# AlibabaResearch/efficientteacher

Measured on AMD Instinct MI355X. Metric: SSOD images/sec (teacher+student step) YOLOv5l 640px, higher is better.
Workload: dtype bf16

## Files before the change

### efficientteacher_amd/csrc/spatial.hip

```cpp
#include "et_host.h"

template <typename T>
__global__ __launch_bounds__(256) void pack_input_kernel(const float* __restrict__ x, T* __restrict__ y, int C, int HW, long long total) {
    const unsigned iu = blockIdx.x * 256u + threadIdx.x;
    if (iu >= total) return;
    const long long i = iu, b = iu / (unsigned)HW, hw = iu - (unsigned)b * (unsigned)HW;
    T v[8];
#pragma unroll
    for (int c = 0; c < 8; ++c) v[c] = et_elem<T>::st(c < C ? x[(b * C + c) * HW + hw] : 0.f);
    T* d = y + i * 8;
#pragma unroll
    for (int c = 0; c < 8; ++c) d[c] = v[c];
}

template <typename T>
__global__ __launch_bounds__(256) void pack_input_u8_kernel(const uint8_t* __restrict__ x, T* __restrict__ y, int C, int HW,
                                                            long long total, float scale) {
    const unsigned iu = blockIdx.x * 256u + threadIdx.x;
    if (iu >= total) return;
    const long long i = iu, b = iu / (unsigned)HW, hw = iu - (unsigned)b * (unsigned)HW;
    T v[8];
#pragma unroll
    for (int c = 0; c < 8; ++c) v[c] = et_elem<T>::st(c < C ? (float)x[(b * C + c) * HW + hw] / scale : 0.f);
    T* d = y + i * 8;
#pragma unroll
    for (int c = 0; c < 8; ++c) d[c] = v[c];
}

template <typename IN, typename T = uint16_t>
__global__ __launch_bounds__(256) void pack_input4_bf16_kernel(const IN* __restrict__ x, T* __restrict__ y, int C, int HW4,
                                                               long long total4, float scale) {
    const unsigned qu = blockIdx.x * 256u + threadIdx.x;
    if (qu >= total4) return;
    const unsigned b = qu / (unsigned)HW4, h4 = qu - b * (unsigned)HW4;
    float v[4][4];
#pragma unroll
    for (int c = 0; c < 4; ++c) {
#pragma unroll
        for (int j = 0; j < 4; ++j) v[c][j] = 0.f;
        if (c < C) {
            const long long off = ((long long)b * C + c) * HW4 * 4 + (long long)h4 * 4;
            if constexpr (sizeof(IN) == 4) {
                const float4 t = *(const float4*)((const float*)x + off);
                v[c][0] = t.x; v[c][1] = t.y; v[c][2] = t.z; v[c][3] = t.w;
            } else {
                const unsigned w = *(const unsigned*)((const uint8_t*)x + off);
#pragma unroll
                for (int j = 0; j < 4; ++j) v[c][j] = (float)((w >> (8 * j)) & 0xffu) / scale;
            }
        }
    }
    T* const d = y + ((long long)b * HW4 * 4 + (long long)h4 * 4) * 8;
#pragma unroll
    for (int j = 0; j < 4; ++j)
        *(uint4*)(d + j * 8) = make_uint4(et_lp<T>::pack(v[0][j], v[1][j]), et_lp<T>::pack(v[2][j], v[3][j]), 0u, 0u);
}

template <typename T> struct PV;
template <> struct PV<float> {
    static constexpr int N = 4;
    __device__ static __forceinline__ void load(const float* p, float (&v)[4]) { const float4 t = *(const float4*)p; v[0] = t.x; v[1] = t.y; v[2] = t.z; v[3] = t.w; }
    __device__ static __forceinline__ void store(float* p, const float (&v)[4]) { *(float4*)p = make_float4(v[0], v[1], v[2], v[3]); }
};
template <typename T> struct PVlp {
    static constexpr int N = 8;
    __device__ static __forceinline__ void load(const T* p, float (&v)[8]) {
        const uint4 t = *(const uint4*)p;
        const unsigned w[4] = {t.x, t.y, t.z, t.w};
#pragma unroll
        for (int i = 0; i < 4; ++i) { v[2 * i] = et_lp<T>::lo(w[i]); v[2 * i + 1] = et_lp<T>::hi(w[i]); }
    }
    __device__ static __forceinline__ void store(T* p, const float (&v)[8]) {
        *(uint4*)p = make_uint4(et_lp<T>::pack(v[0], v[1]), et_lp<T>::pack(v[2], v[3]), et_lp<T>::pack(v[4], v[5]), et_lp<T>::pack(v[6], v[7]));
    }
};
template <> struct PV<uint16_t> : PVlp<uint16_t> {};
template <> struct PV<et_f16> : PVlp<et_f16> {};

template <typename T>
__global__ __launch_bounds__(256) void maxpool5_fwd_kernel(const T* __restrict__ x, int ldx, T* __restrict__ y, int ldy,
                                                           unsigned char* __restrict__ idx, int H, int W, int CV, long long total) {
    constexpr int N = PV<T>::N;
    const unsigned iu = blockIdx.x * 256u + threadIdx.x;
    if (iu >= total) return;
    const unsigned pu = iu / (unsigned)CV, tu = pu / (unsigned)W;
    const int cv = (int)(iu - pu * (unsigned)CV);
    const long long p = pu;
    const int ox = (int)(pu - tu * (unsigned)W);
    const long long b = tu / (unsigned)H;
    const int oy = (int)(tu - (unsigned)b * (unsigned)H);
    float best[N];
    unsigned char bi[N];
#pragma unroll
    for (int k = 0; k < N; ++k) { best[k] = -INFINITY; bi[k] = 0; }
    for (int ky = 0; ky < 5; ++ky) {
        const int iy = oy + ky - 2;
        if ((unsigned)iy >= (unsigned)H) continue;
        for (int kx = 0; kx < 5; ++kx) {
            const int ix = ox + kx - 2;
            if ((unsigned)ix >= (unsigned)W) continue;
            float v[N];
            PV<T>::load(x + ((b * H + iy) * W + ix) * ldx + cv * N, v);
#pragma unroll
            for (int k = 0; k < N; ++k)
                if (v[k] > best[k]) { best[k] = v[k]; bi[k] = (unsigned char)(ky * 5 + kx); }
        }
    }
    PV<T>::store(y + p * ldy + cv * N, best);
    unsigned char* ip = idx + (p * CV + cv) * N;
#pragma unroll
    for (int k = 0; k < N; ++k) ip[k] = bi[k];
}

template <typename T>
__global__ __launch_bounds__(256) void maxpool5_bwd_kernel(const T* __restrict__ dy, int lddy, const unsigned char* __restrict__ idx,
                                                           const T* __restrict__ base, int ldb, T* __restrict__ dx, int lddx,
                                                           int H, int W, int CV, long long total) {
    constexpr int N = PV<T>::N;
    const unsigned iu = blockIdx.x * 256u + threadIdx.x;
    if (iu >= total) return;
    const unsigned pu = iu / (unsigned)CV, tu = pu / (unsigned)W;
    const int cv = (int)(iu - pu * (unsigned)CV);
    const long long p = pu;
    const int ix = (int)(pu - tu * (unsigned)W);
    const long long b = tu / (unsigned)H;
    const int iy = (int)(tu - (unsigned)b * (unsigned)H);
    float acc[N];
    if (base) PV<T>::load(base + p * ldb + cv * N, acc);
    else {
#pragma unroll
        for (int k = 0; k < N; ++k) acc[k] = 0.f;
    }
    for (int ky = 0; ky < 5; ++ky) {
        const int oy = iy - ky + 2;
        if ((unsigned)oy >= (unsigned)H) continue;
        for (int kx = 0; kx < 5; ++kx) {
            const int ox = ix - kx + 2;
            if ((unsigned)ox >= (unsigned)W) continue;
            const long long q = (b * H + oy) * W + ox;
            float g[N];
            PV<T>::load(dy + q * lddy + cv * N, g);
            const unsigned char* ip = idx + (q * CV + cv) * N;
            const unsigned char code = (unsigned char)(ky * 5 + kx);
#pragma unroll
            for (int k = 0; k < N; ++k)
                if (ip[k] == code) acc[k] += g[k];
        }
    }
    PV<T>::store(dx + p * lddx + cv * N, acc);
}

template <typename T>
__global__ __launch_bounds__(256) void upsample2x_fwd_kernel(const T* __restrict__ x, int ldx, T* __restrict__ y, int ldy, int H, int W,
                                                             int CV, long long total) {
    const unsigned iu = blockIdx.x * 256u + threadIdx.x;
    if (iu >= total) return;
    const unsigned pu = iu / (unsigned)CV, tu = pu / (unsigned)(2 * W);
    const int cv = (int)(iu - pu * (unsigned)CV);
    const long long p = pu;
    const int ox = (int)(pu - tu * (unsigned)(2 * W));
    const long long b = tu / (unsigned)(2 * H);
    const int oy = (int)(tu - (unsigned)b * (unsigned)(2 * H));
    const uint4 v = *(const uint4*)((const char*)(x + ((b * H + (oy >> 1)) * W + (ox >> 1)) * ldx) + (size_t)cv * 16);
    *(uint4*)((char*)(y + p * ldy) + (size_t)cv * 16) = v;
}

template <typename T>
__global__ __launch_bounds__(256) void upsample2x_bwd_kernel(const T* __restrict__ dy, int lddy, T* __restrict__ dx, int lddx, int H, int W,
                                                             int CV, long long total, int accumulate) {
    constexpr int N = PV<T>::N;
    const unsigned iu = blockIdx.x * 256u + threadIdx.x;
    if (iu >= total) return;
    const unsigned pu = iu / (unsigned)CV, tu = pu / (unsigned)W;
    const int cv = (int)(iu - pu * (unsigned)CV);
    const long long p = pu;
    const int w = (int)(pu - tu * (unsigned)W);
    const long long b = tu / (unsigned)H;
    const int h = (int)(tu - (unsigned)b * (unsigned)H);
    float acc[N];
    if (accumulate) PV<T>::load(dx + p * lddx + cv * N, acc);
    else {
#pragma unroll
        for (int k = 0; k < N; ++k) acc[k] = 0.f;
    }
#pragma unroll
    for (int d = 0; d < 4; ++d) {
        const long long q = (b * 2 * H + (2 * h + (d >> 1))) * 2 * W + (2 * w + (d & 1));
        float g[N];
        PV<T>::load(dy + q * lddy + cv * N, g);
#pragma unroll
        for (int k = 0; k < N; ++k) acc[k] += g[k];
    }
    PV<T>::store(dx + p * lddx + cv * N, acc);
}

extern "C" int et_pack_input(const float* x_nchw, void* y_nhwc8, int dtype, int B, int C, int H, int W, et_stream_t stream) {
    if (!x_nchw || !y_nhwc8) return -1;
    if (B <= 0 || C <= 0 || C > 8 || H <= 0 || W <= 0) return -2;
    const long long total = (long long)B * H * W;
    if (total >= (1ll << 31)) return -2;
    return with_dtype(dtype, [&](auto t) {
        using T = typename decltype(t)::type;
        const bool quads = et_is_lp<T>::value && C <= 4 && (H * W) % 4 == 0 && ((((uintptr_t)x_nchw) | ((uintptr_t)y_nhwc8)) & 15) == 0;
        if constexpr (et_is_lp<T>::value) {
            if (quads)
                hipLaunchKernelGGL((pack_input4_bf16_kernel<float, T>), dim3(et_cdiv(total / 4, 256)), dim3(256), 0, (hipStream_t)stream, x_nchw,
                                   (T*)y_nhwc8, C, H * W / 4, total / 4, 1.0f);
        }
        if (!quads)
            hipLaunchKernelGGL((pack_input_kernel<T>), dim3(et_cdiv(total, 256)), dim3(256), 0, (hipStream_t)stream, x_nchw, (T*)y_nhwc8, C, H * W, total);
        ET_CHECK_LAUNCH();
        return 0;
    });
}

extern "C" int et_pack_input_u8(const uint8_t* x_nchw, void* y_nhwc8, int dtype, int B, int C, int H, int W, float norm_scale,
                                et_stream_t stream) {
    if (!x_nchw || !y_nhwc8) return -1;
    if (B <= 0 || C <= 0 || C > 8 || H <= 0 || W <= 0 || !(norm_scale > 0.f)) return -2;
    const long long total = (long long)B * H * W;
    if (total >= (1ll << 31)) return -2;
    return with_dtype(dtype, [&](auto t) {
        using T = typename decltype(t)::type;
        const bool quads = et_is_lp<T>::value && C <= 4 && (H * W) % 4 == 0 && (((uintptr_t)x_nchw) & 3) == 0 && (((uintptr_t)y_nhwc8) & 15) == 0;
        if constexpr (et_is_lp<T>::value) {
            if (quads)
                hipLaunchKernelGGL((pack_input4_bf16_kernel<uint8_t, T>), dim3(et_cdiv(total / 4, 256)), dim3(256), 0, (hipStream_t)stream, x_nchw,
                                   (T*)y_nhwc8, C, H * W / 4, total / 4, norm_scale);
        }
        if (!quads)
            hipLaunchKernelGGL((pack_input_u8_kernel<T>), dim3(et_cdiv(total, 256)), dim3(256), 0, (hipStream_t)stream, x_nchw, (T*)y_nhwc8, C, H * W, total,
                               norm_scale);
        ET_CHECK_LAUNCH();
        return 0;
    });
}

extern "C" int et_maxpool5_fwd(const void* x, int ldx, void* y, int ldy, uint8_t* argmax, int dtype, int B, int H, int W, int C,
                               et_stream_t stream) {
    if (!x || !y || !argmax) return -1;
    const int vec = et_vec(dtype), CV = C / vec;
    if (B <= 0 || !et_whole_vecs(vec, C, ldx, ldy)) return -2;
    const long long total = (long long)B * H * W * CV;
    if (total >= (1ll << 31)) return -2;
    return with_dtype(dtype, [&](auto t) {
        using T = typename decltype(t)::type;
        hipLaunchKernelGGL((maxpool5_fwd_kernel<T>), dim3(et_cdiv(total, 256)), dim3(256), 0, (hipStream_t)stream, (const T*)x, ldx, (T*)y, ldy, argmax,
                           H, W, CV, total);
        ET_CHECK_LAUNCH();
        return 0;
    });
}

extern "C" int et_maxpool5_bwd(const void* dy, int lddy, const uint8_t* argmax, const void* base, int ldb, void* dx, int lddx,
                               int dtype, int B, int H, int W, int C, et_stream_t stream) {
    if (!dy || !dx || !argmax) return -1;
    const int vec = et_vec(dtype), CV = C / vec;
    if (B <= 0 || !et_whole_vecs(vec, C, lddy, lddx) || (base && ldb % vec)) return -2;
    const long long total = (long long)B * H * W * CV;
    if (total >= (1ll << 31)) return -2;
    return with_dtype(dtype, [&](auto t) {
        using T = typename decltype(t)::type;
        hipLaunchKernelGGL((maxpool5_bwd_kernel<T>), dim3(et_cdiv(total, 256)), dim3(256), 0, (hipStream_t)stream, (const T*)dy, lddy, argmax,
                           (const T*)base, ldb, (T*)dx, lddx, H, W, CV, total);
        ET_CHECK_LAUNCH();
        return 0;
    });
}

extern "C" int et_upsample2x_fwd(const void* x, int ldx, void* y, int ldy, int dtype, int B, int H, int W, int C, et_stream_t stream) {
    if (!x || !y) return -1;
    const int vec = et_vec(dtype), CV = C / vec;
    if (B <= 0 || !et_whole_vecs(vec, C, ldx, ldy)) return -2;
    const long long total = (long long)B * 4 * H * W * CV;
    if (total >= (1ll << 31)) return -2;
    return with_dtype(dtype, [&](auto t) {
        using T = typename decltype(t)::type;
        hipLaunchKernelGGL((upsample2x_fwd_kernel<T>), dim3(et_cdiv(total, 256)), dim3(256), 0, (hipStream_t)stream, (const T*)x, ldx, (T*)y, ldy, H, W,
                           CV, total);
        ET_CHECK_LAUNCH();
        return 0;
    });
}

extern "C" int et_upsample2x_bwd(const void* dy, int lddy, void* dx, int lddx, int dtype, int B, int H, int W, int C, int accumulate,
                                 et_stream_t stream) {
    if (!dy || !dx) return -1;
    const int vec = et_vec(dtype), CV = C / vec;
    if (B <= 0 || !et_whole_vecs(vec, C, lddy, lddx)) return -2;
    const long long total = (long long)B * H * W * CV;
    if (total >= (1ll << 31)) return -2;
    return with_dtype(dtype, [&](auto t) {
        using T = typename decltype(t)::type;
        hipLaunchKernelGGL((upsample2x_bwd_kernel<T>), dim3(et_cdiv(total, 256)), dim3(256), 0, (hipStream_t)stream, (const T*)dy, lddy, (T*)dx, lddx,
                           H, W, CV, total, accumulate);
        ET_CHECK_LAUNCH();
        return 0;
    });
}
```

Before: 1344.

## Use register-tiled sliding-window maxpool5 forward and backward kernels for 16-bit types

Replaces the per-output-pixel 5x5 maxpool (used in SPPF) with a tiled kernel. Each thread walks a 5-row by 2-column tile for 4 channels, keeping a 4-row ring of column maxima in registers so input rows are reused rather than reloaded 25 times. Values are encoded as order-preserving integer keys with position bits packed in, so a single unsigned max yields both the value and the argmax. The backward pass scatters gradients with a sliding accumulator ring in the same way. The cost is heavy register pressure and intricate bit-encoding logic, and the change only matters for the few SPPF pooling layers in the step.

```diff
diff --git a/efficientteacher_amd/csrc/spatial.hip b/efficientteacher_amd/csrc/spatial.hip
--- a/efficientteacher_amd/csrc/spatial.hip
+++ b/efficientteacher_amd/csrc/spatial.hip
@@ -148,6 +148,201 @@
         }
     }
     PV<T>::store(dx + p * lddx + cv * N, acc);
+}
+
+constexpr int POOL_R = 5, POOL_S = 2, POOL_V = 4;
+
+template <int NW> __device__ __forceinline__ void pool_ld(const void* p, unsigned (&w)[NW]) {
+    static_assert(NW == 1 || NW == 2 || NW == 4, "4, 8 or 16 bytes");
+    if constexpr (NW == 4) { const uint4 t = *(const uint4*)p; w[0] = t.x; w[1] = t.y; w[2] = t.z; w[3] = t.w; }
+    else if constexpr (NW == 2) { const uint2 t = *(const uint2*)p; w[0] = t.x; w[1] = t.y; }
+    else w[0] = *(const unsigned*)p;
+}
+template <int NW> __device__ __forceinline__ void pool_st(void* p, const unsigned (&w)[NW]) {
+    static_assert(NW == 1 || NW == 2 || NW == 4, "4, 8 or 16 bytes");
+    if constexpr (NW == 4) *(uint4*)p = make_uint4(w[0], w[1], w[2], w[3]);
+    else if constexpr (NW == 2) *(uint2*)p = make_uint2(w[0], w[1]);
+    else *(unsigned*)p = w[0];
+}
+__device__ __forceinline__ unsigned pool_max3(unsigned a, unsigned b, unsigned c) {
+    const unsigned m = a > b ? a : b;
+    return m > c ? m : c;
+}
+struct PoolTile { long long b; int y0, x0, cv; };
+template <int R, int S>
+__device__ __forceinline__ bool pool_tile(int H, int W, int CV, unsigned total, PoolTile& t) {
+    const unsigned iu = blockIdx.x * 256u + threadIdx.x;
+    if (iu >= total) return false;
+    const unsigned TY = (unsigned)(H + R - 1) / R, TX = (unsigned)(W + S - 1) / S;
+    const unsigned tu = iu / (unsigned)CV, ru = tu / TX, b = ru / TY;
+    t.cv = (int)(iu - tu * (unsigned)CV);
+    t.x0 = (int)(tu - ru * TX) * S;
+    t.y0 = (int)(ru - b * TY) * R;
+    t.b = b;
+    return true;
+}
+
+template <typename T, int R, int S, int V>
+__global__ __launch_bounds__(256) void maxpool5_tile_fwd_kernel(const T* __restrict__ x, int ldx, T* __restrict__ y, int ldy,
+                                                                unsigned char* __restrict__ idx, int H, int W, int CV, unsigned total) {
+    static_assert(sizeof(T) == 2 && V % 4 == 0 && R + 4 <= 32 && S + 4 <= 16, "16-bit elements; 9 position bits");
+    constexpr int NW = V / 2, HC = S + 4;
+    PoolTile t;
+    if (!pool_tile<R, S>(H, W, CV, total, t)) return;
+    long long xrow = ((t.b * H + (t.y0 - 2)) * W + (t.x0 - 2)) * ldx + t.cv * V;
+    long long yrow = ((t.b * H + t.y0) * W + t.x0) * ldy + t.cv * V, irow = (((t.b * H + t.y0) * W + t.x0) * CV + t.cv) * V;
+    bool colin[HC];
+#pragma unroll
+    for (int c = 0; c < HC; ++c) colin[c] = (unsigned)(t.x0 - 2 + c) < (unsigned)W;
+    unsigned ring[4][S][V];
+#pragma unroll
+    for (int a = 0; a < 4; ++a)
+#pragma unroll
+        for (int s = 0; s < S; ++s)
+#pragma unroll
+            for (int v = 0; v < V; ++v) ring[a][s][v] = 0u;
+#pragma unroll 1
+    for (int j = 0; j < R + 4; ++j) {
+        const bool rowin = (unsigned)(t.y0 - 2 + j) < (unsigned)H;
+        unsigned k[HC][V];
+#pragma unroll
+        for (int c = 0; c < HC; ++c) {
+            const bool in = rowin && colin[c];
+            unsigned w[NW];
+#pragma unroll
+            for (int i = 0; i < NW; ++i) w[i] = 0u;
+            if (in) pool_ld<NW>(x + xrow + (long long)c * ldx, w);
+#pragma unroll
+            for (int i = 0; i < NW; ++i) {
+                const unsigned m = (w[i] >> 15) & 0x00010001u;
+                const unsigned k16 = (w[i] ^ (m * 0xffffu | 0x80008000u)) + m;
+                const unsigned low = (unsigned)(511 - (16 * j + c)) << 2 | ((m | m >> 15) & 3u);
+                k[c][2 * i] = in ? (k16 << 16 | low) : 0u;
+                k[c][2 * i + 1] = in ? ((k16 & 0xffff0000u) | low) : 0u;
+            }
+        }
+        unsigned cur[S][V];
+#pragma unroll
+        for (int s = 0; s < S; ++s)
+#pragma unroll
+            for (int v = 0; v < V; ++v) cur[s][v] = pool_max3(pool_max3(k[s][v], k[s + 1][v], k[s + 2][v]), k[s + 3][v], k[s + 4][v]);
+        if (j >= 4) {
+            const int r = j - 4;
+#pragma unroll
+            for (int s = 0; s < S; ++s) {
+                unsigned val[NW], code[NW / 2];
+#pragma unroll
+                for (int i = 0; i < NW / 2; ++i) code[i] = 0u;
+#pragma unroll
+                for (int v = 0; v < V; ++v) {
+                    const unsigned m = pool_max3(pool_max3(ring[0][s][v], ring[1][s][v], ring[2][s][v]), ring[3][s][v], cur[s][v]);
+                    const unsigned k16 = m & 0xffff0000u, p = (~m >> 2) & 511u;
+                    const unsigned bits = (m & (1u << (v & 1))) ? 0u - k16 : k16 ^ 0x80000000u;
+                    val[v / 2] = (v & 1) ? (val[v / 2] | bits) : bits >> 16;
+                    code[v / 4] |= (p - 11u * (p >> 4) - (unsigned)(5 * r + s)) << (8 * (v & 3));
+                }
+                if (t.y0 + r < H && colin[s + 2]) {
+                    pool_st<NW>(y + yrow + (long long)s * ldy, val);
+                    pool_st<NW / 2>(idx + irow + (long long)s * CV * V, code);
+                }
+            }
+            yrow += (long long)W * ldy;
+            irow += (long long)W * CV * V;
+        }
+        xrow += (long long)W * ldx;
+#pragma unroll
+        for (int s = 0; s < S; ++s)
+#pragma unroll
+            for (int v = 0; v < V; ++v) {
+                ring[0][s][v] = ring[1][s][v]; ring[1][s][v] = ring[2][s][v]; ring[2][s][v] = ring[3][s][v]; ring[3][s][v] = cur[s][v];
+            }
+    }
+}
+
+template <typename T, int R, int S, int V>
+__global__ __launch_bounds__(256) void maxpool5_tile_bwd_kernel(const T* __restrict__ dy, int lddy, const unsigned char* __restrict__ idx,
+                                                                const T* __restrict__ base, int ldb, T* __restrict__ dx, int lddx,
+                                                                int H, int W, int CV, unsigned total) {
+    static_assert(sizeof(T) == 2 && V % 4 == 0, "16-bit elements, whole index words");
+    constexpr int NW = V / 2, HC = S + 4;
+    PoolTile t;
+    if (!pool_tile<R, S>(H, W, CV, total, t)) return;
+    long long grow = ((t.b * H + (t.y0 + R + 1)) * W + (t.x0 - 2)) * lddy + t.cv * V;
+    long long irow = (((t.b * H + (t.y0 + R + 1)) * W + (t.x0 - 2)) * CV + t.cv) * V;
+    long long brow = ((t.b * H + (t.y0 + R - 1)) * W + t.x0) * ldb + t.cv * V, xrow = ((t.b * H + (t.y0 + R + 3)) * W + t.x0) * lddx + t.cv * V;
+    bool colin[HC];
+#pragma unroll
+    for (int c = 0; c < HC; ++c) colin[c] = (unsigned)(t.x0 - 2 + c) < (unsigned)W;
+    float acc[5][S][V];
+#pragma unroll
+    for (int a = 0; a < 5; ++a)
+#pragma unroll
+        for (int s = 0; s < S; ++s)
+#pragma unroll
+            for (int v = 0; v < V; ++v) acc[a][s][v] = 0.f;
+#pragma unroll 1
+    for (int j = R + 3; j >= 0; --j) {
+        const bool rowin = (unsigned)(t.y0 - 2 + j) < (unsigned)H;
+        float g[HC][V];
+        unsigned code[HC][NW / 2];
+#pragma unroll
+        for (int c = 0; c < HC; ++c) {
+            unsigned w[NW];
+#pragma unroll
+            for (int i = 0; i < NW; ++i) w[i] = 0u;
+#pragma unroll
+            for (int i = 0; i < NW / 2; ++i) code[c][i] = 0xffffffffu;
+            if (rowin && colin[c]) {
+                pool_ld<NW>(dy + grow + (long long)c * lddy, w);
+                pool_ld<NW / 2>(idx + irow + (long long)c * CV * V, code[c]);
+            }
+#pragma unroll
+            for (int i = 0; i < NW; ++i) { g[c][2 * i] = et_lp<T>::lo(w[i]); g[c][2 * i + 1] = et_lp<T>::hi(w[i]); }
+        }
+        if (j >= 4) {
+#pragma unroll
+            for (int s = 0; s < S; ++s) {
+                unsigned w[NW];
+#pragma unroll
+                for (int i = 0; i < NW; ++i) w[i] = 0u;
+                if (base && t.y0 + j - 4 < H && colin[s + 2]) pool_ld<NW>(base + brow + (long long)s * ldb, w);
+#pragma unroll
+                for (int i = 0; i < NW; ++i) { acc[0][s][2 * i] = et_lp<T>::lo(w[i]); acc[0][s][2 * i + 1] = et_lp<T>::hi(w[i]); }
+            }
+        }
+#pragma unroll
+        for (int a = 0; a < 5; ++a) {
+            if (j - 4 + a < 0 || j - 4 + a >= R) continue;
+#pragma unroll
+            for (int s = 0; s < S; ++s)
+#pragma unroll
+                for (int kx = 0; kx < 5; ++kx)
+#pragma unroll
+                    for (int v = 0; v < V; ++v) {
+                        const bool hit = ((code[s + 4 - kx][v / 4] >> (8 * (v & 3))) & 0xffu) == (unsigned)(a * 5 + kx);
+                        acc[a][s][v] += hit ? g[s + 4 - kx][v] : -0.0f;
+                    }
+        }
+        if (j < R) {
+#pragma unroll
+            for (int s = 0; s < S; ++s) {
+                unsigned w[NW];
+#pragma unroll
+                for (int i = 0; i < NW; ++i) w[i] = et_lp<T>::pack(acc[4][s][2 * i], acc[4][s][2 * i + 1]);
+                if (t.y0 + j < H && colin[s + 2]) pool_st<NW>(dx + xrow + (long long)s * lddx, w);
+            }
+        }
+        grow -= (long long)W * lddy;
+        irow -= (long long)W * CV * V;
+        brow -= (long long)W * ldb;
+        xrow -= (long long)W * lddx;
+#pragma unroll
+        for (int a = 4; a > 0; --a)
+#pragma unroll
+            for (int s = 0; s < S; ++s)
+#pragma unroll
+                for (int v = 0; v < V; ++v) acc[a][s][v] = acc[a - 1][s][v];
+    }
 }
 
 template <typename T>
@@ -245,8 +440,13 @@
     if (total >= (1ll << 31)) return -2;
     return with_dtype(dtype, [&](auto t) {
         using T = typename decltype(t)::type;
-        hipLaunchKernelGGL((maxpool5_fwd_kernel<T>), dim3(et_cdiv(total, 256)), dim3(256), 0, (hipStream_t)stream, (const T*)x, ldx, (T*)y, ldy, argmax,
-                           H, W, CV, total);
+        if constexpr (et_is_lp<T>::value) {
+            const long long tiles = (long long)B * et_cdiv(H, POOL_R) * et_cdiv(W, POOL_S) * (C / POOL_V);
+            hipLaunchKernelGGL((maxpool5_tile_fwd_kernel<T, POOL_R, POOL_S, POOL_V>), dim3(et_cdiv(tiles, 256)), dim3(256), 0, (hipStream_t)stream,
+                               (const T*)x, ldx, (T*)y, ldy, argmax, H, W, C / POOL_V, (unsigned)tiles);
+        } else
+            hipLaunchKernelGGL((maxpool5_fwd_kernel<T>), dim3(et_cdiv(total, 256)), dim3(256), 0, (hipStream_t)stream, (const T*)x, ldx, (T*)y, ldy,
+                               argmax, H, W, CV, total);
         ET_CHECK_LAUNCH();
         return 0;
     });
@@ -261,8 +461,13 @@
     if (total >= (1ll << 31)) return -2;
     return with_dtype(dtype, [&](auto t) {
         using T = typename decltype(t)::type;
-        hipLaunchKernelGGL((maxpool5_bwd_kernel<T>), dim3(et_cdiv(total, 256)), dim3(256), 0, (hipStream_t)stream, (const T*)dy, lddy, argmax,
-                           (const T*)base, ldb, (T*)dx, lddx, H, W, CV, total);
+        if constexpr (et_is_lp<T>::value) {
+            const long long tiles = (long long)B * et_cdiv(H, POOL_R) * et_cdiv(W, POOL_S) * (C / POOL_V);
+            hipLaunchKernelGGL((maxpool5_tile_bwd_kernel<T, POOL_R, POOL_S, POOL_V>), dim3(et_cdiv(tiles, 256)), dim3(256), 0, (hipStream_t)stream,
+                               (const T*)dy, lddy, argmax, (const T*)base, ldb, (T*)dx, lddx, H, W, C / POOL_V, (unsigned)tiles);
+        } else
+            hipLaunchKernelGGL((maxpool5_bwd_kernel<T>), dim3(et_cdiv(total, 256)), dim3(256), 0, (hipStream_t)stream, (const T*)dy, lddy, argmax,
+                               (const T*)base, ldb, (T*)dx, lddx, H, W, CV, total);
         ET_CHECK_LAUNCH();
         return 0;
     });
```

After: 1351 (median of 6 runs). About the same (+0.5%).
